# wondras/ld-decode

Hardware: AMD Instinct MI355X
Metric: RF Msamples/s (40 MSPS NTSC, full RF->.tbc decode) (higher is better)
Workload: dtype f64

## Files before the change

### ld-decode_amd/csrc/abi.inc

```
#include <hip/hip_runtime.h>
#include <algorithm>
#include <chrono>
#include <thread>
#include <cmath>
#include <complex>
#include <cstdio>
#include <cstring>
#include <map>
#include <string>
#include <vector>

namespace {

using namespace ldg;

struct DevBuf {
  void* p = nullptr;
  size_t n = 0;
};

}

static inline comb::CombOpt comb_defaults() {
  comb::CombOpt c;
// ... 801 lines not shown
  return LDG_OK;
}

int ldg_set_capture(ldg_ctx* ctx, const void* data, int64_t nsamples, int fmt, int64_t first_sample,
                    int is_device) {
  if (!ctx || !data || nsamples <= 0 || fmt < 0 || fmt > 3 || first_sample < 0) return LDG_EINVAL;
  if ((fmt == 2 && first_sample % 3) || (fmt == 3 && first_sample % 4)) return LDG_EINVAL;
  LDG_TRY(hipSetDevice(ctx->device));
  if (int rc = ldg_stream_close(ctx)) return rc;
  ctx->cap_ring = 0;
  size_t nbytes;
  switch (fmt) {
    case 0: nbytes = (size_t)nsamples; break;
    case 1: nbytes = (size_t)nsamples * 2; break;
    case 2: nbytes = (size_t)((nsamples + 2) / 3) * 4; break;
    default: nbytes = (size_t)((nsamples + 3) / 4) * 5; break;
  }
  if (is_device) {
    if (ctx->cap_owned) dfree(ctx->cap);
    ctx->cap = (uint8_t*)data;
    ctx->cap_owned = false;
    ctx->cap_alloc = nbytes;
  } else {
    if (!ctx->cap_owned || ctx->cap_alloc < nbytes) {
      if (ctx->cap_owned) dfree(ctx->cap);
      ctx->cap = nullptr;
      int rc = dmalloc(ctx, &ctx->cap, nbytes + 16);
      if (rc) return rc;
      ctx->cap_alloc = nbytes;
      ctx->cap_owned = true;
    }
    LDG_TRY(hipMemcpy(ctx->cap, data, nbytes, hipMemcpyHostToDevice));
  }
  ctx->fmt = fmt;
  ctx->cap_first = first_sample;
  ctx->cap_nsamp = nsamples;
  return LDG_OK;
}

static int stream_prepare(ldg_ctx* ctx, hipStream_t s, int64_t hi);

static int64_t steady_ns() {
  return std::chrono::duration_cast<std::chrono::nanoseconds>(std::chrono::steady_clock::now().time_since_epoch())
      .count();
}
static unsigned long long* span_slot(ldg_ctx* ctx) {
  if (!ctx->prof_on || !ctx->d_span || ctx->span_n >= ldg_ctx::SPAN_MAX) return nullptr;
  ctx->span_issue_ns.push_back(steady_ns());
  return ctx->d_span + 2 * (size_t)ctx->span_n++;
}

static int launch_demod(ldg_ctx* ctx, hipStream_t st, int n, const int32_t* M_) {
  const SysConst C = ctx->C;
  LDG_LAUNCH_ON(st, "demod", ldg_k_demod, n * MAX_BLOCKS_PER_READ, 1024, M_, ctx->d_reads, ctx->cap, ctx->cap_first,
             ctx->cap_nsamp, ctx->cap_ring, ctx->fmt, ctx->tw, ctx->twk, ctx->rf_cur, ctx->fvideo, ctx->f05, ctx->iirtab, ctx->alf, ctx->arf, C, ctx->video, ctx->vread, ctx->vchan,
             ctx->d_status, ctx->d_ospill, ++ctx->park_epoch, ctx->d_stile, ctx->d_aslice,
             ctx->d_sst, ctx->d_sbits, ctx->d_bst, span_slot(ctx));
  return check_launch(ctx, "ldg_k_demod");
}

static int launch_chain(ldg_ctx* ctx, hipStream_t st, int n, const int32_t* M_) {
  const SysConst C = ctx->C;
  if (!(ctx->skip >> 0 & 1)) LDG_LAUNCH_ON(st, "sync_walk", ldg_k_sync_walk, n * SEG_K, 64, M_, ctx->d_reads, ctx->video, ctx->vread, ctx->vchan, C,
             ctx->d_status, ctx->d_npos, ctx->d_npk, ctx->d_nlv, ctx->d_ncnt, ctx->d_stile, ctx->d_sst,
             ctx->d_sbits);
  if (!(ctx->skip >> 1 & 1)) LDG_LAUNCH_ON(st, "sync", ldg_k_sync, n, 64, M_, ctx->d_reads, ctx->video, ctx->vread, ctx->vchan, C, ctx->d_recs,
             ctx->d_peaks, ctx->d_status, ctx->d_npos, ctx->d_npk, ctx->d_nlv, ctx->d_ncnt, ctx->d_stile,
             ctx->d_sst, ctx->d_sbits, (ctx->skip >> 9) & 1);
  if (!(ctx->skip >> 2 & 1)) LDG_LAUNCH_ON(st, "linelocs", ldg_k_linelocs, n, 64, M_, ctx->video, ctx->vread, ctx->vchan, C, ctx->d_recs,
             ctx->d_peaks, ctx->d_lines, ctx->d_bad, ctx->d_sst, ctx->d_sbits);
  const dim3 g_lines((unsigned)(C.frame_lines / 2 + 5), (unsigned)n), g_rows((unsigned)(C.frame_lines / 2 + 1), (unsigned)n);
  if (!(ctx->skip >> 3 & 1)) LDG_LAUNCH_ON(st, "hsync_lines", ldg_k_hsync_lines, g_lines, 64, M_, ctx->video, ctx->vread, ctx->vchan, C,
             ctx->d_recs, ctx->d_lines, ctx->d_bad, ctx->d_reads);
  if (!(ctx->skip >> 4 & 1)) LDG_LAUNCH_ON(st, "hsync_field", ldg_k_hsync_field, n, 256, M_, C, ctx->d_recs, ctx->d_lines, ctx->d_bad);
  if (!(ctx->skip >> 5 & 1)) LDG_LAUNCH_ON(st, "philips", ldg_k_philips, n, 192, M_, ctx->video, ctx->vread, ctx->vchan, C, ctx->d_recs,
             ctx->d_lines, ctx->d_reads);
  if (int rc = check_launch(ctx, "field kernels")) return rc;
  if (ctx->system == 0) {
    for (int pass = 0; pass < 2; pass++) {
      if (!(ctx->skip >> 6 & 1)) LDG_LAUNCH_ON(st, "burst_lines", ldg_k_burst_lines, g_lines, 64, M_, ctx->video, ctx->vread, ctx->vchan, C,
                 ctx->d_recs, ctx->d_lines, ctx->d_blevel, pass, ctx->d_bst, ctx->d_reads);
      if (!(ctx->skip >> 7 & 1)) LDG_LAUNCH_ON(st, "burst_field", ldg_k_burst_field, n, 64, M_, ctx->video, ctx->vread, ctx->vchan,
                 ctx->d_recs, ctx->d_lines, ctx->d_blevel, C, pass, ctx->d_bst, ctx->d_reads);
    }
  } else {
    LDG_LAUNCH_ON(st, "pilot_lines", ldg_k_pilot_lines, g_lines, 64, M_, ctx->video, ctx->vread, ctx->vchan, C,
               ctx->d_recs, ctx->d_lines, ctx->d_scratch, ctx->d_reads);
    LDG_LAUNCH_ON(st, "pilot_field", ldg_k_pilot_field, n, 256, M_, ctx->d_recs, ctx->d_lines, C, ctx->d_scratch,
               ctx->d_reads);
  }
  if (!(ctx->skip >> 8 & 1)) {
    if (C.hz_ire_r != 0.0)
      LDG_LAUNCH_ON(st, "final_lines", ldg_k_final_lines, g_rows, FINAL_NT, M_, ctx->video, ctx->vread, ctx->vchan, C,
                    ctx->d_recs, ctx->d_lines, ctx->d_blevel, ctx->d_pic, ctx->pic_stride, ctx->d_reads);
    else
      LDG_LAUNCH_ON(st, "final_lines", ldg_k_final_lines_div, g_rows, FINAL_NT, M_, ctx->video, ctx->vread, ctx->vchan, C,
                    ctx->d_recs, ctx->d_lines, ctx->d_blevel, ctx->d_pic, ctx->pic_stride, ctx->d_reads);
  }
  if (int rc = check_launch(ctx, "tbc kernels")) return rc;
  return LDG_OK;
}

struct HostProf {
  bool on = getenv("LDG_HOSTPROF") != nullptr;
  std::chrono::steady_clock::time_point t0 = std::chrono::steady_clock::now(), t = t0;
  char buf[512];
  int len = 0;
// ... 144 lines not shown
    ctx->rf_tab[ci] = nullptr;
    ctx->rf_cap[ci] = 0;
    if (int rc = dmalloc(ctx, &ctx->rf_tab[ci], (size_t)want * BLOCKLEN)) return rc;
    ctx->rf_cap[ci] = want;
  }
  ctx->rf_cur = ctx->rf_tab[ci];
  if (ctx->cs && (ctx->stages & 1)) {
    int64_t hi = 0;
    for (int i = 0; i < n; i++) {
      const int64_t w = (full && (full[i] & LDG_READ_PROBE)) ? probe_halfwin(ctx->C) : 0;
      hi = std::max(hi, nr[i].s0 + (int64_t)(nr[i].n_blocks - 1) * BLOCKSTEP + BLOCKLEN + w);
    }
    if (int rc = stream_prepare(ctx, s, hi)) return rc;
  }
  ReadDesc* hpr = (ReadDesc*)(ctx->h_probe + (size_t)ci * R * (sizeof(ReadDesc) + sizeof(int32_t)));
  int32_t* hps = (int32_t*)(hpr + R);
  int np = 0;
  if (full)
    for (int i = 0; i < n; i++) {
      if (!(full[i] & LDG_READ_PROBE)) continue;
      ReadDesc pr = nr[i];
      const int64_t r0 = nr[i].readsample - PROBE_C;
      if (!(ctx->stages & 1) || r0 - BLOCKCUT < ctx->cap_first ||
          r0 - BLOCKCUT + BLOCKLEN > ctx->cap_first + ctx->cap_nsamp) {
        full[i] &= (uint8_t)~LDG_READ_PROBE;
        continue;
      }
      read_geometry(pr, r0);
      pr.end = r0 + BLOCKSTEP + 64;
      pr.n_out = (int32_t)(pr.end - pr.s0 + 1);
      pr.n_blocks = 1;
      pr.n_audio = (int32_t)((pr.end - pr.s0) / AUDIO_DIV1 + 1);
      pr.n_audio2 = pr.n_audio / AUDIO_DIV2;
      pr.vcut = 0;
      pr.acut1 = pr.acut2 = ACUT_NONE;
      hpr[np] = pr;
      hps[np++] = smap[i];
    }
  int32_t* dps = ctx->d_psm + (size_t)ci * R;
  hipStream_t sp = ctx->sprep;
  if (call.demod_recorded) LDG_TRY(hipStreamWaitEvent(sp, call.ev_demod, 0));
  LDG_LAUNCH_ON(sp, "new_reads", ldg_k_new_reads, (n + 255) / 256, 256, hnr, hsm, n, dsm, ctx->d_reads, ctx->d_status);
  if (np) LDG_LAUNCH_ON(sp, "new_reads", ldg_k_new_reads, (np + 255) / 256, 256, hpr, hps, np, dps, ctx->d_preads,
                        ctx->d_status);
    LDG_LAUNCH_ON(sp, "rf_table", ldg_k_rf_table, dim3(BLOCKLEN / 256, (unsigned)tm.size()), 256, ctx->rfvideo, ctx->mtf,
                  ctx->mtf_logabs, ctx->mtf_arg, htm, ctx->rf_cur);
  if (int rc = check_launch(ctx, "ldg_k_rf_table")) return rc;
  LDG_TRY(hipEventRecord(call.ev_prep, sp));
  LDG_TRY(hipStreamWaitEvent(s, call.ev_prep, 0));
  if (ctx->frames_recorded && ctx->frames_demod) LDG_TRY(hipStreamWaitEvent(s, ctx->ev_frames, 0));
  hp_.mark("prep");
  if (np && (ctx->stages & 1)) {
    const SysConst C = ctx->C;
    LDG_LAUNCH_ON(s, "demod_probe", ldg_k_demod_probe, np, 1024, dps, ctx->d_preads, ctx->cap, ctx->cap_first,
                  ctx->cap_nsamp, ctx->cap_ring, ctx->fmt, ctx->tw, ctx->twk, ctx->rf_cur, ctx->fvideo, ctx->f05, ctx->iirtab,
                  ctx->alf, ctx->arf, C, ctx->video, ctx->vread, ctx->vchan,
                  ctx->d_status, ctx->d_ospill, ++ctx->park_epoch, ctx->d_stile, ctx->d_aslice, ctx->d_sst,
                  ctx->d_sbits, ctx->d_bst, nullptr);
    LDG_LAUNCH_ON(s, "probe_pick", ldg_k_probe_pick, np, 64, dps, ctx->d_preads, ctx->d_reads, ctx->d_status,
                  ctx->d_sst, ctx->d_sbits, C, probe_halfwin(C));
    if (int rc = check_launch(ctx, "ldg_k_probe_pick")) return rc;
    ctx->probes += np;
  }
  const int ng = (ctx->stages & 4) ? std::max(1, std::min(ctx->nsub, n / 4)) : 0;
  auto group = [&](int g, int& i0, int& m) {
    i0 = (int)((int64_t)n * g / ng);
    m = (int)((int64_t)n * (g + 1) / ng) - i0;
  };
  if (ctx->stages & 1)
    if (int rc = launch_demod(ctx, s, n, dsm)) return rc;
  hp_.mark("demod");
  LDG_TRY(hipEventRecord(call.ev_demod, s));
  call.demod_recorded = true;
  LDG_TRY(hipStreamWaitEvent(ctx->sa, call.ev_demod, 0));
  if (ctx->audio_recorded) LDG_TRY(hipStreamWaitEvent(ctx->sa, ctx->ev_audio, 0));
  if (ctx->stages & 2) LDG_LAUNCH_ON(ctx->sa, "audio1", ldg_k_audio1, n * MAX_BLOCKS_PER_READ, A1_T, dsm, ctx->d_reads,
                                     ctx->tw, ctx->C, ctx->d_aslice, ctx->audio1, ctx->a1read, ctx->a1chan, ctx->d_status);
  if (ctx->stages & 2) LDG_LAUNCH_ON(ctx->sa, "audio2", ldg_k_audio2, n * AUDIO2_WG, 1024, dsm, ctx->d_reads, ctx->tw, ctx->lpf2, ctx->audio1,
                ctx->a1read, ctx->a1chan, ctx->audio2, ctx->a2read, ctx->a2chan, ctx->d_status);
  if (int rc = check_launch(ctx, "ldg_k_audio2")) return rc;
  LDG_TRY(hipEventRecord(call.ev_done[0], ctx->sa));
  hp_.mark("audio");
  int nd = 1;
  for (int g = 0; g < ng; g++) {
    int i0, m;
    group(g, i0, m);
    if (m <= 0) continue;
    hipStream_t st = ctx->sub[g];
    LDG_TRY(hipStreamWaitEvent(st, call.ev_demod, 0));
    if (ctx->frames_recorded) LDG_TRY(hipStreamWaitEvent(st, ctx->ev_frames, 0));
    if (ctx->audio_recorded) LDG_TRY(hipStreamWaitEvent(st, ctx->ev_audio, 0));
    if (int rc = launch_chain(ctx, st, m, dsm + i0)) return rc;
    LDG_TRY(hipEventRecord(call.ev_done[nd++], st));
  hp_.mark("chain");
  }
  call.ndone = nd;
  for (int k = 0; k < nd; k++) LDG_TRY(hipStreamWaitEvent(ctx->srec, call.ev_done[k], 0));
  call.seq = ++ctx->seq;
  LDG_LAUNCH_ON(ctx->srec, "recs_out", ldg_k_recs_out, 1, 256, ctx->d_recs, dsm, n, ctx->d_reads,
                ctx->h_recs_pin + (size_t)ci * R,
                ctx->h_done + ci, call.seq);
  LDG_TRY(hipEventRecord(call.ev_copied, ctx->srec));
  hp_.mark("rec");
  call.n = n;
  call.smap = smap;
  for (int i = 0; i < n; i++) {
    ctx->h_reads[smap[i]] = nr[i];
// ... 831 lines not shown
  if (ctx->pal_state) {
    const double init2[2] = {-1.0, -1.0};
    LDG_TRY(hipMemcpy(ctx->pal_state, init2, sizeof(init2), hipMemcpyHostToDevice));
    ctx->pal_scur = 0;
  }
  return LDG_OK;
}

int ldg_comb_set_state(ldg_ctx* ctx, double aburstlev) {
  if (!ctx) return LDG_EINVAL;
  LDG_TRY(hipSetDevice(ctx->device));
  if (int rc = comb_quiesce(ctx)) return rc;
  if (int rc = comb_alloc(ctx)) return rc;
  LDG_TRY(hipMemcpy(ctx->comb_state, &aburstlev, sizeof(double), hipMemcpyHostToDevice));
  return LDG_OK;
}

int ldg_demod_isolated_ex(ldg_ctx* ctx, int n, const int32_t* slots, int iters, int variant, double* ms_per_launch) {
  if (!ctx || !slots || n <= 0 || n > ctx->max_reads || iters <= 0 || !ms_per_launch) return LDG_EINVAL;
  if (variant != 0 && variant != 1) return LDG_EINVAL;
  for (int i = 0; i < n; i++)
    if (slots[i] < 0 || slots[i] >= ctx->max_reads || !ctx->live[slots[i]]) return LDG_EINVAL;
  LDG_TRY(hipSetDevice(ctx->device));
  LDG_TRY(hipDeviceSynchronize());
  if (!ctx->d_isomap) {
    if (int rc = dmalloc(ctx, &ctx->d_isomap, (size_t)ctx->max_reads)) return rc;
  }
  LDG_TRY(hipMemcpy(ctx->d_isomap, slots, (size_t)n * sizeof(int32_t), hipMemcpyHostToDevice));
  std::vector<int32_t> st_h((size_t)ctx->max_reads);
  LDG_TRY(hipMemcpy(st_h.data(), ctx->d_status, st_h.size() * sizeof(int32_t), hipMemcpyDeviceToHost));
  for (int i = 0; i < n; i++)
    if (st_h[slots[i]] == FS_EOF) { ctx->err = "demod_isolated: a read lies outside the resident capture"; return LDG_ESTATE; }
  if (!ctx->rf_cur) { ctx->err = "demod_isolated: no decode yet"; return LDG_ESTATE; }
  int nt = 1;
  for (int i = 0; i < n; i++) nt = std::max(nt, ctx->h_reads[slots[i]].filt_slot + 1);
  if (ctx->rf_iso_cap < nt) {
    dfree(ctx->rf_iso);
    ctx->rf_iso = nullptr;
    ctx->rf_iso_cap = 0;
    if (int rc = dmalloc(ctx, &ctx->rf_iso, (size_t)nt * BLOCKLEN)) return rc;
    ctx->rf_iso_cap = nt;
  }
  for (int t = 0; t < nt; t++)
    LDG_TRY(hipMemcpy(ctx->rf_iso + (size_t)t * BLOCKLEN, ctx->rf_cur, BLOCKLEN * sizeof(double2),
                      hipMemcpyDeviceToDevice));
  const SysConst C = ctx->C;
  hipStream_t st = ctx->stream;
  std::vector<hipEvent_t> ev(2 * (size_t)iters, nullptr);
  int rc = LDG_OK;
  auto step = [&](hipError_t e) { if (!rc && e != hipSuccess) { ctx->err = hipGetErrorString(e); rc = LDG_EDEVICE; } };
  for (auto& e : ev) step(hipEventCreate(&e));
  for (int k = 0; k < iters && !rc; k++) {
    step(hipEventRecord(ev[2 * k], st));
    (variant ? ldg_k_demod_iso_cut : ldg_k_demod_iso)<<<n * MAX_BLOCKS_PER_READ, 1024, 0, st>>>(
          ctx->d_isomap, ctx->d_reads, ctx->cap, ctx->cap_first, ctx->cap_nsamp, ctx->cap_ring, ctx->fmt, ctx->tw, ctx->twk,
          ctx->rf_iso, ctx->fvideo, ctx->f05, ctx->iirtab, ctx->alf, ctx->arf, C,
          ctx->video, ctx->vread, ctx->vchan, ctx->d_status, ctx->d_ospill,
          ++ctx->park_epoch, ctx->d_stile, ctx->d_aslice, ctx->d_sst, ctx->d_sbits, ctx->d_bst, nullptr);
    step(hipEventRecord(ev[2 * k + 1], st));
  }
  if (!rc) rc = check_launch(ctx, variant ? "ldg_k_demod_iso_cut" : "ldg_k_demod_iso");
  if (!rc) step(hipStreamSynchronize(st));
  double tot = 0;
  for (int k = 0; k < iters && !rc; k++) {
    float ms = 0;
    step(hipEventElapsedTime(&ms, ev[2 * k], ev[2 * k + 1]));
    tot += ms;
  }
  if (!rc) {
    *ms_per_launch = tot / iters;
    step(hipMemcpy(st_h.data(), ctx->d_status, st_h.size() * sizeof(int32_t), hipMemcpyDeviceToHost));
    for (int i = 0; i < n && !rc; i++)
      if (st_h[slots[i]] == FS_EOF) { ctx->err = "demod_isolated: a read returned FS_EOF"; rc = LDG_ESTATE; }
  }
  for (auto& e : ev)
    if (e) (void)hipEventDestroy(e);
  return rc;
}

int ldg_demod_isolated(ldg_ctx* ctx, int n, const int32_t* slots, int iters, double* ms_per_launch) {
  return ldg_demod_isolated_ex(ctx, n, slots, iters, 0, ms_per_launch);
}

int ldg_sync(ldg_ctx* ctx) {
  if (!ctx) return LDG_EINVAL;
  LDG_TRY(hipSetDevice(ctx->device));
  for (hipStream_t st : {ctx->stream2, ctx->scomb, ctx->stream, ctx->stream_b, ctx->sa, ctx->sout, ctx->srec, ctx->sprep}) LDG_TRY(hipStreamSynchronize(st));
  for (int k = 0; k < ctx->nsub; k++) LDG_TRY(hipStreamSynchronize(ctx->sub[k]));
  ctx->comb_pending = false;
  ctx->out_head = ctx->out_n = 0;
  prof_collect(ctx);
  return LDG_OK;
}

int ldg_comb_async(ldg_ctx* ctx, int n) {
  if (!ctx || n < 0 || n > ctx->max_frames) return LDG_EINVAL;
  if (!ctx->have_filters) { ctx->err = "comb: set the filters (the system) first"; return LDG_ESTATE; }
  if (n == 0) return LDG_OK;
  if (ctx->C.system == 0) return ldg_comb_ntsc_async(ctx, n);
  LDG_TRY(hipSetDevice(ctx->device));
  if (int rc = pal_alloc(ctx)) return rc;
  hipStream_t c = ctx->scomb;
  const int b = ctx->fb;
  LDG_TRY(hipStreamWaitEvent(c, ctx->ev_frames, 0));
  if (int rc = pal_launch(ctx, c, ctx->frame_buf(b), n)) return rc;
  LDG_TRY(hipEventRecord(ctx->ev_fbuf[b], c));
  ctx->fbuf_recorded[b] = true;
// ... 721 lines not shown
```

### ld-decode_amd/csrc/demod.hip

```cpp
#include <hip/hip_runtime.h>
#include <type_traits>
#include "common.hpp"
#include "fft8k.hpp"
#include "iir.hpp"
#include "chan.hpp"
#include "tail.hpp"
#include "sample.hpp"

using namespace ldg;

namespace {

constexpr int T = 1024;
constexpr int M = HALF;

__device__ __forceinline__ double2 rsplit(double2 A, double2 B, double2 w) {
  const double2 e = make_double2(0.5 * (A.x + B.x), 0.5 * (A.y - B.y));
  const double2 d = make_double2(A.x - B.x, A.y + B.y);
  const double2 o = make_double2(0.5 * d.y, -0.5 * d.x);
  return cadd(e, cmul(w, o));
}

__device__ __forceinline__ double2 cmerge(double2 Pk, double2 Pkp, double2 w) {
  const double2 e = make_double2(0.5 * (Pk.x + Pkp.x), 0.5 * (Pk.y - Pkp.y));
// ... 37 lines not shown
  } else if (z < 252) {
    p = 32 + (z - 248);
    pp = 39 - (z - 248);
  } else if (z < 255) {
    p = z - 251;
    pp = 8 - p;
  } else if (z == 255) {
    return {0, 0, M};
  } else {
    return {4, 4, 4};
  }
  return {p, pp, pp};
}

static_assert(sizeof(double2) * HALF > 160 * 1024 / 2, "demod workgroups must not share a CU");
__device__ __forceinline__ int cu_slot() {
  const unsigned hw = __builtin_amdgcn_s_getreg((31 << 11) | 4);
  const unsigned xcc = __builtin_amdgcn_s_getreg((31 << 11) | 20);
  return (int)(((xcc & 7u) << 8) | (((hw >> 13) & 7u) << 5) | (((hw >> 12) & 1u) << 4) | ((hw >> 8) & 15u));
}

__device__ __forceinline__ int fresh(int tid) { asm volatile("" : "+v"(tid)); return tid; }

__device__ __forceinline__ bool pair_live(int tid, int c) { return c < 4 || tid == 0; }

__device__ __forceinline__ double2 tw_mirror(double2 w) { return make_double2(-w.x, w.y); }

#ifdef LDG_PROBE
constexpr int kProbe = LDG_PROBE;
#else
constexpr int kProbe = 0;
#endif
#ifdef LDG_PROBE_NOSTORE
constexpr bool kProbeNoStore = true;
#else
constexpr bool kProbeNoStore = false;
#endif

__device__ __forceinline__ void st_pair(double* a, double2 z) {
  typedef double v2d __attribute__((ext_vector_type(2)));
  const v2d zv = {z.x, z.y};
  __builtin_nontemporal_store(zv, reinterpret_cast<v2d*>(a));
}
__device__ __forceinline__ void st_park(double2* a, double2 z) { *a = z; }
__device__ __forceinline__ unsigned long long* park_owner(double2* ospill) {
  return reinterpret_cast<unsigned long long*>(ospill + (int64_t)PARK_TOTAL * M);
}
__device__ __forceinline__ int uni(int v) { return __builtin_amdgcn_readfirstlane(v); }
template <class T> __device__ __forceinline__ T* at32(T* base, int i) {
  using B = std::conditional_t<std::is_const<T>::value, const char, char>;
  return reinterpret_cast<T*>(reinterpret_cast<B*>(base) + (uint32_t)i * (uint32_t)sizeof(T));
}

__device__ __forceinline__ void store_wave(char* ob, uint32_t voff, int lo, int l2, double2 z, int copylen) {
  double* const a = reinterpret_cast<double*>(ob + voff);
  if (lo >= BLOCKCUT && lo + 127 < BLOCKCUT + copylen) {
    st_pair(a, z);
  } else if (lo + 127 >= BLOCKCUT && lo < BLOCKCUT + copylen) {
    const int p = lo + l2;
    const bool in0 = p >= BLOCKCUT && p < BLOCKCUT + copylen;
    const bool in1 = p + 1 >= BLOCKCUT && p + 1 < BLOCKCUT + copylen;
    if (in0 && in1) *reinterpret_cast<double2*>(a) = z;
    else if (in0) a[0] = z.x;
    else if (in1) a[1] = z.y;
  }
}

struct LaneStore {
  uint32_t voff;
  int wlo;
  int l2;
};
__device__ __forceinline__ LaneStore lane_store(int t) { return {16u * (uint32_t)t, uni(2 * (t & ~63)), 2 * (t & 63)}; }
__device__ __forceinline__ void store_q(double* o, LaneStore ls, int q, double2 z, int copylen) {
  store_wave(reinterpret_cast<char*>(o) + 16384 * q, ls.voff, ls.wlo + 2048 * q, ls.l2, z, copylen);
}

__device__ __forceinline__ void store_chan(const double2* sx, double* o, int t, int copylen) {
  if (kProbeNoStore) return;
  const LaneStore ls = lane_store(t);
#pragma unroll
  for (int q = 0; q < 8; q++) {
    const int m = t + 1024 * q;
    store_q(o, ls, q, sx[SWC(m)], copylen);
  }
}

__device__ __forceinline__ bool am_beats32(double v, int vi, double b, int bi) {
  const bool vn = v != v, bn = b != b;
  if (vn || bn) return vn && (!bn || vi < bi);
  return v > b || (v == b && vi < bi);
}

__constant__ double c_atan64[65] = {
    0.0, 0.015623728620476831, 0.031239833430268277, 0.046840712915969654,
    0.06241880999595735, 0.0779666338315423, 0.09347678115858947, 0.1089419569898658,
    0.12435499454676144, 0.13970887428916365, 0.15499674192394097, 0.1702119252854744,
    0.18534794999569476, 0.2003985538258785, 0.21535769969773805, 0.23021958727684372,
    0.24497866312686414, 0.2596296294082575, 0.2741674511196588, 0.2885873618940774,
    0.3028848683749714, 0.31705575320914703, 0.3310960767041321, 0.34500217720710513,
    0.35877067027057225, 0.3723984466767542, 0.38588266939807375, 0.39922076957525254,
    0.4124104415973873, 0.42544963737004227, 0.43833655985795783, 0.4510696559885235,
    0.4636476090008061, 0.4760693303227612, 0.48833395105640554, 0.5004408131472942,
    0.5123894603107377, 0.5241796287829132, 0.5358112379604637, 0.5472843809874369,
    0.5585993153435624, 0.5697564534829784, 0.5807563535676704, 0.5915997103351114,
    0.6022873461349642, 0.6128202021652414, 0.6231993299340659, 0.6334258829691446,
// ... 44 lines not shown
}

__device__ __forceinline__ void merge_pairs(const CBuf x, const double2* __restrict__ twk,
                                            const double2* __restrict__ G, int tid, const Pairs& D) {
  tid = fresh(tid);
#pragma unroll
  for (int c = 0; c < 5; c++) {
    if (!pair_live(tid, c)) continue;
    const Slot sl = slot_of(tid, c);
    const double2 wk = *at32(twk, sl.p);
    const double2 Pk = cmul(D.a[c], *at32(G, sl.p));
    const double2 Pkp = cmul(D.b[c], *at32(G, sl.gp));
    x[sl.p] = cmerge(Pk, Pkp, wk);
    if (sl.pp != sl.p) x[sl.pp] = cmerge(Pkp, Pk, tw_mirror(wk));
  }
}

}

#ifdef LDG_STAMPS
constexpr int LDG_STAMP_BLOCKS = 8192;
__device__ unsigned long long g_stamps[LDG_STAMP_BLOCKS][32];
#define STAMP(i)                                                                   \
  do {                                                                             \
    __syncthreads();                                                               \
    if (threadIdx.x == 0 && blockIdx.x < LDG_STAMP_BLOCKS)                         \
      g_stamps[blockIdx.x][i] = __builtin_readcyclecounter();                      \
  } while (0)
#else
#define STAMP(i) \
  do {           \
  } while (0)
#endif

#define LDG_DEMOD_ARG_LIST(P, V, L)                                                                    \
  P(const int32_t, smap) P(const ReadDesc, reads) P(const uint8_t, cap) V(int64_t, cap_first)         \
  V(int64_t, cap_nsamp) V(int64_t, ring) V(int, fmt) P(const double2, tw) P(const double2, twk)       \
  P(const double2, rf_filt) P(const double2, g_video) P(const double2, g_05) P(const double, iir)     \
  P(const double2, a_lfilt) P(const double2, a_rfilt) V(SysConst, C) P(double, video)                 \
  V(int64_t, vread_stride) V(int64_t, vchan_stride) P(int32_t, status) P(double2, ospill)             \
  V(unsigned long long, park_epoch) P(SyncTile, stiles) P(double2, aslice) P(double, sst)             \
  P(uint32_t, sbits) P(double4, bst) L(unsigned long long, span)
#define LDG_DEMOD_PARAMS LDG_KERNEL_PARAMS(LDG_DEMOD_ARG_LIST)
struct DemodKargs {
  LDG_KARG_FIELDS(LDG_DEMOD_ARG_LIST)
};
#define DK(name) LDG_KARG(DemodKargs, name)
#define DKP(name) LDG_KARG_PTR(DemodKargs, name)
static_assert(alignof(SysConst) == 8 && offsetof(DemodKargs, fmt) == 48 && offsetof(DemodKargs, tw) == 56 &&
                  offsetof(DemodKargs, C) == 120 && offsetof(DemodKargs, video) == 120 + sizeof(SysConst) &&
                  offsetof(DemodKargs, span) == 208 + sizeof(SysConst) && sizeof(DemodKargs) == 216 + sizeof(SysConst),
              "DemodKargs is the kernels' argument list");
#define LDG_DEMOD_ARGS LDG_KERNEL_ARGS(LDG_DEMOD_ARG_LIST)
template <bool CUT, bool PROBE = false>
__device__ __forceinline__ void demod_body(LDG_DEMOD_PARAMS) {
  __shared__ double2 s_x[M];
  __shared__ uint16_t s_bits[BLOCKLEN / 16];
  __shared__ double2 s_tw[TW_LDS_N];
  __shared__ IIRAux s_aux;
  __shared__ double s_atan[65];
  const CBuf X_{s_x};
  const int tid = threadIdx.x;
  if (tid < 65) s_atan[tid] = c_atan64[tid];
  s_tw[tw_lds_pos(tid)] = tw[2 * tid];
  const TwLds twl{s_tw};
  const FftLane fl = fft_lane(tid);
  STAMP(0);
  if (unsigned long long* const span = DKP(span); span && tid == 0)
    atomicMax(&span[0], ~(unsigned long long)__builtin_amdgcn_s_memrealtime());
  const int slot = PROBE ? smap[blockIdx.x] : smap[blockIdx.x / MAX_BLOCKS_PER_READ];
  const int b = PROBE ? 0 : blockIdx.x % MAX_BLOCKS_PER_READ;
  const ReadDesc rd = reads[slot];
  if (b >= rd.n_blocks) return;

  const int64_t i0 = rd.s0 + (int64_t)b * BLOCKSTEP;
  const int off = b * BLOCKSTEP;
  const int copylen = (off + (BLOCKLEN - BLOCKCUT) > rd.n_out) ? rd.n_out - off : BLOCKSTEP;
  int64_t rel0 = i0 - cap_first;
  if (rel0 < 0 || rel0 + BLOCKLEN > cap_nsamp) {
    if (tid == 0) DKP(status)[slot] = FS_EOF;
    return;
  }
  if (ring) {
    const int spg = fmt == 2 ? 3 : fmt == 3 ? 4 : 1, bpg = fmt == 1 ? 2 : fmt == 2 ? 4 : fmt == 3 ? 5 : 1;
    const int64_t g = i0 / spg;
    cap += (g * bpg) % ring;
    rel0 = i0 - g * spg;
  }
  auto vout = [&](int ch) {
    return DKP(video) + (int64_t)slot * DK(vread_stride) + off - BLOCKCUT + (int64_t)ch * DK(vchan_stride);
  };
  const double2* F = rf_filt + (int64_t)rd.filt_slot * BLOCKLEN;
  __shared__ int s_park;
  const int my_cu = cu_slot();
  unsigned long long* const owners = park_owner(ospill);
  const unsigned long long my_tag = (park_epoch << 32) | (unsigned long long)blockIdx.x;
  int my_park = -1;
  if (tid == 0) {
    if (atomicCAS(owners + my_cu, 0ull, my_tag) == 0ull) my_park = my_cu;
    for (int e = 0; e < PARK_EXTRA && my_park < 0; e++) {
      const int u = PARK_SLOTS + ((my_cu + e) & (PARK_EXTRA - 1));
      if (atomicCAS(owners + u, 0ull, my_tag) == 0ull) my_park = u;
    }
    s_park = my_park;
  }
  constexpr double TAU = 6.283185307179586;

  if (fmt == 0 || fmt == 1) {
    double x[16];
    if (fmt == 0) {
      uint4 w;
      __builtin_memcpy(&w, at32(cap + rel0, 16 * tid), 16);
      const uint32_t wd[4] = {w.x, w.y, w.z, w.w};
#pragma unroll
      for (int i = 0; i < 16; i++) x[i] = (double)((wd[i >> 2] >> (8 * (i & 3))) & 0xffu);
    } else {
      uint4 w[2];
      __builtin_memcpy(w, at32(reinterpret_cast<const int16_t*>(cap) + rel0, 16 * tid), 32);
      const uint32_t wd[8] = {w[0].x, w[0].y, w[0].z, w[0].w, w[1].x, w[1].y, w[1].z, w[1].w};
#pragma unroll
      for (int i = 0; i < 16; i++) x[i] = (double)(int16_t)(wd[i >> 1] >> (16 * (i & 1)));
    }
#pragma unroll
    for (int r = 0; r < 8; r++) X_[8 * tid + r] = make_double2(x[2 * r], x[2 * r + 1]);
  } else {
#pragma unroll
    for (int q = 0; q < 8; q++) {
      const int m = tid + T * q;
      X_[m] = make_double2(load_sample(cap, fmt, rel0 + 2 * m), load_sample(cap, fmt, rel0 + 2 * m + 1));
    }
  }
  STAMP(1);
  if (!(kProbe & 8)) fft8k_dif<false>(s_x, tw, twl, tid, fl);
  else __syncthreads();
  STAMP(2);
  const int park_id = uni(s_park);
  const bool park_lost = park_id < 0;
  double2* const park = ospill + (int64_t)(park_lost ? PARK_SCRATCH : park_id) * M;
  auto finish = [&] {
    if (tid == 0 && park_lost) DKP(status)[slot] = FS_MIGRATED;
    if (unsigned long long* const span = DKP(span); span && tid == 0)
      atomicMax(&span[1], (unsigned long long)__builtin_amdgcn_s_memrealtime());
  };

  {
    Pairs X;
    if (!(kProbe & 64)) split_pairs(X_, twk, tid, X);
    else for (int c = 0; c < 5; c++) { X.a[c] = X_[tid + 1024 * c]; X.b[c] = X.a[c]; }
    if (!(CUT && a1_block_dead(b, rd.acut1))) {
      const int t = fresh(tid);
      const int a0 = DK(C).audio_lo0;
      const bool mir = t >= 512;
      const int k = mir ? a0 + 1 + (t - 512) : a0 + t;
      const int j = mir ? a0 + 1024 - k : t;
      double2 xk = rsplit(X_[dr_pos(k)], X_[dr_pos(M - k)], *at32(tw, k));
      if (mir) xk = conj2(xk);
      const double2 al = cmul(xk, *at32(DKP(a_lfilt), j)), ar = cmul(xk, *at32(DKP(a_rfilt), j));
      double2* as = DKP(aslice) + ((int64_t)slot * MAX_BLOCKS_PER_READ + b) * 2048;
      *at32(as, j) = al;
      *at32(as + 1024, j) = ar;
    }
    __syncthreads();
    const int t = fresh(tid);
#pragma unroll
    for (int c = 0; c < 5; c++) {
      if (!pair_live(t, c) || (kProbe & 16)) continue;
      const Slot sl = slot_of(t, c);
      auto Fv = [&](int i) { return (kProbe & 128) ? make_double2(1.0 + i * 1e-9, 0.5) : *at32(F, i); };
      const double2 wk = *at32(twk, sl.p);
      const double2 yk = cmul(X.a[c], Fv(sl.p));
      const double2 yk2 = cmul(conj2(X.b[c]), Fv(M + sl.p));
      X_[sl.p] = cadd(yk, yk2);
      if (!(kProbe & 256)) {
        const double2 o = cmulc(csub(yk, yk2), wk);
        st_park(at32(park, SW(sl.p)), o);
      }
      if (sl.pp != sl.p) {
        const double2 ykp = cmul(X.b[c], Fv(sl.pp));
        const double2 ykp2 = cmul(conj2(X.a[c]), Fv(M + sl.pp));
        X_[sl.pp] = cadd(ykp, ykp2);
        if (!(kProbe & 256)) st_park(at32(park, SW(sl.pp)), cmulc(csub(ykp, ykp2), tw_mirror(wk)));
      }
    }
  }

  STAMP(3);
  double the[8], tho[8];
#pragma clang loop unroll(disable)
  for (int h = 0; h < 2; h++) {
    STAMP(4 + 2 * h);
    if (h == 1 && tid == 0 && my_park >= 0)
      __hip_atomic_store(owners + my_park, 0ull, __ATOMIC_RELAXED, __HIP_MEMORY_SCOPE_AGENT);
    double2 zr[8];
    fft8k_dit<true, true>(s_x, tw, twl, tid, zr, fl);
    if (h == 0) {
      asm volatile("s_waitcnt vmcnt(0)" ::: "memory");
      __syncthreads();
      const int t = fresh(tid);
      const int wbase = __builtin_amdgcn_readfirstlane(t & ~63);
#pragma unroll
      for (int i = 0; i < 8; i++)
        __builtin_amdgcn_global_load_lds((const void*)at32(park + T * i, t),
                                         (__attribute__((address_space(3))) void*)(s_x + T * i + wbase), 16, 0, 0);
    }
    STAMP(5 + 2 * h);
#pragma unroll
    for (int q = 0; q < 8; q++) {
      const double2 z = zr[q];
      const double a = (kProbe & 1) ? z.y * 0.5 + z.x : kFastAtan2 ? fast_atan2(z.y, z.x, s_atan) : atan2(z.y, z.x);
      if (h) tho[q] = a;
      else the[q] = a;
    }
    asm volatile("s_waitcnt vmcnt(0)" ::: "memory");
    __syncthreads();

  }
  double* ph = reinterpret_cast<double*>(s_x);
#pragma unroll
  for (int q = 0; q < 8; q++) ph[tid + T * q] = tho[q];
  __syncthreads();

  STAMP(8);
  {
    const double hzk = DK(C).freq_hz / TAU;
    double d0[8], d1[8];
#pragma unroll
    for (int q = 0; q < 8; q++) {
      const int m = tid + T * q;
      const double prev = m ? ph[m - 1] : 0.0;
      d0[q] = m ? fold_tau(the[q] - prev) * hzk : 0.0;
      d1[q] = fold_tau(tho[q] - the[q]) * hzk;
    }
    __syncthreads();
#pragma unroll
    for (int q = 0; q < 8; q++) X_[tid + T * q] = make_double2(d0[q], d1[q]);
  }
  STAMP(9);
  fft8k_dif<false>(s_x, tw, twl, tid, fl);
  STAMP(10);
  Pairs D;
  if (!(kProbe & 64)) split_pairs(X_, twk, tid, D);
  else for (int c = 0; c < 5; c++) { D.a[c] = X_[tid + 1024 * c]; D.b[c] = D.a[c]; }
  __syncthreads();
  STAMP(11);

  const double inv = 1.0 / (double)M;
  double pl1, pt1, p151, p311;
  double2* sx = s_x;
  {
    if (!(kProbe & 32)) merge_pairs(X_, twk, DKP(g_05), tid, D);
    STAMP(12);
    double2 zr[8];
    fft8k_dit<true, true>(s_x, tw, twl, tid, zr, fl);
    STAMP(13);
    const int t = fresh(tid);
    pl1 = *at32(iir + IIR_P1, t & 63);
    pt1 = *at32(iir + IIR_P1, t);
    p151 = *at32(iir + IIR_P1, scan_d15(t & 63));
    p311 = *at32(iir + IIR_P1, scan_d31(t & 63));
    double* o = vout(CH_05) - BLOCKCUT_END;
    const double sync_lo = DK(C).sync_lo, sync_hi = DK(C).sync_hi;
    LaneStore ls = lane_store(t);
    ls.wlo -= BLOCKCUT_END;
    const bool st05 = !kProbeNoStore && !(CUT && (int64_t)off >= rd.vcut);
#pragma unroll
    for (int q = 0; q < 8; q++) {
      const int m = t + T * q;
      const double v0 = zr[q].x * inv, v1 = zr[q].y * inv;
      if (st05) store_q(o, ls, q, make_double2(v0, v1), copylen);
      const uint32_t f0 = (v0 >= sync_lo && v0 <= sync_hi) ? 1u : 0u;
      const uint32_t f1 = (v1 >= sync_lo && v1 <= sync_hi) ? 1u : 0u;
      int xb = (int)((f0 | (f1 << 1)) << (2 * (t & 7)));
      xb |= __builtin_amdgcn_mov_dpp(xb, 0x111, 0xf, 0xf, true);
      xb |= __builtin_amdgcn_mov_dpp(xb, 0x112, 0xf, 0xf, true);
      xb |= __builtin_amdgcn_mov_dpp(xb, 0x114, 0xf, 0xf, true);
      if ((t & 7) == 7) s_bits[m >> 3] = (uint16_t)xb;
    }
  }
  __syncthreads();
  STAMP(14);
  {
    const int t = fresh(tid);
    const uint32_t cur = s_bits[(t + 2) & 1023], prv = (uint32_t)s_bits[(t + 1) & 1023] >> 15;
    double y[IIR_CHUNK];
    double st_in = 0.0;
    if (!(kProbe & 4)) iir1_bits(cur, prv, iir, &s_aux, t, pl1, pt1, p151, p311, y, &st_in);
    else for (int i = 0; i < IIR_CHUNK; i++) y[i] = (double)((cur >> i) & 1) * pl1;
    const int64_t cbase = (int64_t)slot * CHUNKS_PER_SLOT + (off >> 4) - BLOCKCUT / 16;
    if (16 * t >= BLOCKCUT && 16 * t < BLOCKCUT + copylen) {
      *at32(DKP(sst) + cbase, t) = st_in;
      *at32(DKP(sbits) + cbase, t) = cur | (prv << 16);
    }
    {
      const int j = (t >> 1) - 32, hf = t & 1;
      const int ntile = (copylen + 31) / 32;
      double v = -__builtin_inf();
      int vi = 0x7fffffff;
      const int n0 = 32 * j;
      if (j >= 0 && j < ntile) {
#pragma unroll
        for (int i = 0; i < IIR_CHUNK; i++) {
          const int e = 16 * hf + i;
          if (e < copylen - 32 * j && am_beats32(y[i], n0 + e, v, vi)) { v = y[i]; vi = n0 + e; }
        }
      }
      const double ov = __shfl_xor(v, 1);
      const int oi = __shfl_xor(vi, 1);
      if (am_beats32(ov, oi, v, vi)) { v = ov; vi = oi; }
      if (j >= 0 && j < ntile && hf == 0) {
        SyncTile tt;
        tt.v = v;
        tt.idx = vi == 0x7fffffff ? 0x7fffffffffffffffLL : (int64_t)off + vi;
        *at32(DKP(stiles) + ((int64_t)slot * STILE_PER_SLOT + (off >> 5) - 32), t >> 1) = tt;
      }
    }
  }
  STAMP(15);
  if (CUT && (int64_t)off >= rd.vcut) {
    finish();
    return;
  }
  double4 mlb, mtb, m15b, m31b;
  {
    if (!(kProbe & 32)) merge_pairs(X_, twk, DKP(g_video), tid, D);
    STAMP(16);
    double2 zr[8];
    if (!(kProbe & 2)) fft8k_dit<true, true>(s_x, tw, twl, tid, zr, fl);
    else { __syncthreads(); for (int q = 0; q < 8; q++) zr[q] = s_x[tid + 1024 * q]; __syncthreads(); }
    STAMP(17);
    const int t = fresh(tid);
    mlb = iir2_pow(iir + IIR_MB, t & 63);
    mtb = iir2_pow(iir + IIR_MB, t);
    m15b = iir2_pow(iir + IIR_MB, scan_d15(t & 63));
    m31b = iir2_pow(iir + IIR_MB, scan_d31(t & 63));
    double* o = vout(CH_DEMOD);
    const LaneStore ls = lane_store(t);
#pragma unroll
    for (int q = 0; q < 8; q++) {
      const int m = t + T * q;
      const double2 z = make_double2(zr[q].x * inv, zr[q].y * inv);
      sx[SWC(m)] = z;
      if (!kProbeNoStore) store_q(o, ls, q, z, copylen);
    }
  }
  __syncthreads();
  STAMP(18);
  {
    const int t = fresh(tid);
    double x[IIR_CHUNK];
#pragma unroll
    for (int c = 0; c < 8; c++) {
      const double2 z = sx[SWC(8 * t + c)];
      x[2 * c] = z.x;
      x[2 * c + 1] = z.y;
    }
    const double2 h = sx[SWC((8 * t - 1) & (M - 1))];
    double y[IIR_CHUNK];
    double2 s_in = make_double2(0.0, 0.0);
    if (!(kProbe & 4)) iir2(x, h.y, h.x, iir + 3, iir + IIR_MB, &s_aux, t, mlb, mtb, m15b, m31b, y, &s_in);
    if (16 * t >= BLOCKCUT && 16 * t < BLOCKCUT + copylen) {
      const int64_t cbase = (int64_t)slot * CHUNKS_PER_SLOT + (off >> 4) - BLOCKCUT / 16;
      *at32(DKP(bst) + cbase, t) = make_double4(s_in.x, s_in.y, h.y, h.x);
    }
    if (DK(C).n_chan > 4) {
      double2 p_in;
      iir2(x, h.y, h.x, iir + 8, iir + IIR_MP, &s_aux, t, iir2_pow(iir + IIR_MP, t & 63), iir2_pow(iir + IIR_MP, t),
           iir2_pow(iir + IIR_MP, scan_d15(t & 63)), iir2_pow(iir + IIR_MP, scan_d31(t & 63)), y, &p_in);
#pragma unroll
      for (int c = 0; c < 8; c++) sx[SWC(8 * t + c)] = make_double2(y[2 * c], y[2 * c + 1]);
      __syncthreads();
      store_chan(sx, vout(CH_PILOT), t, copylen);
    }
  }
  STAMP(19);
  finish();
}

extern "C" __global__ __launch_bounds__(1024) void ldg_k_demod(LDG_DEMOD_PARAMS) { demod_body<true>(LDG_DEMOD_ARGS); }

extern "C" __global__ __launch_bounds__(1024) void ldg_k_demod_iso(LDG_DEMOD_PARAMS) { demod_body<false>(LDG_DEMOD_ARGS); }
extern "C" __global__ __launch_bounds__(1024) void ldg_k_demod_iso_cut(LDG_DEMOD_PARAMS) { demod_body<true>(LDG_DEMOD_ARGS); }

constexpr int PROBE_C = BLOCKSTEP / 2;

extern "C" __global__ __launch_bounds__(1024) void ldg_k_demod_probe(LDG_DEMOD_PARAMS) {
  demod_body<true, true>(LDG_DEMOD_ARGS);
}

extern "C" __global__ __launch_bounds__(64) void ldg_k_probe_pick(const int32_t* __restrict__ psm,
                                                                 const ReadDesc* __restrict__ preads,
                                                                 ReadDesc* __restrict__ reads,
                                                                 int32_t* __restrict__ status,
                                                                 const double* __restrict__ sst,
                                                                 const uint32_t* __restrict__ sbits, SysConst C,
                                                                 int halfwin) {
  const int slot = psm[blockIdx.x];
  const int lane = threadIdx.x;
  const bool eof = status[slot] == FS_EOF;
  const SyncSrc ds(sst, sbits, slot, C);
  double best = -1.0;
  int bi = 0x7fffffff;
  if (!eof) {
    for (int o = PROBE_C - halfwin + lane; o <= PROBE_C + halfwin; o += 64) {
      const double v = ds[o];
      if (v > best) { best = v; bi = o; }
    }
  }
#pragma unroll
  for (int m = 1; m < 64; m <<= 1) {
    const double ov = __shfl_xor(best, m);
    const int oi = __shfl_xor(bi, m);
    if (ov > best || (ov == best && oi < bi)) { best = ov; bi = oi; }
  }
  if (lane == 0) {
    if (!eof && best > 0.2) {
      ReadDesc r = reads[slot];
      const int64_t start = preads[slot].readsample + bi;
      r.readsample = start;
      r.end = start + READLEN + 1;
      r.s0 = start > BLOCKCUT ? start - BLOCKCUT : 0;
      r.n_out = (int32_t)(r.end - r.s0 + 1);
      r.n_blocks = (int32_t)((r.end - r.s0 + BLOCKSTEP - 1) / BLOCKSTEP);
      r.n_audio = (int32_t)((r.end - r.s0) / AUDIO_DIV1 + 1);
      r.n_audio2 = r.n_audio / AUDIO_DIV2;
      const TailPlan tp = tail_plan(r.n_audio, r.n_audio2, r.vcut);
      r.acut1 = tp.acut1;
      r.acut2 = tp.acut2;
      if (r.n_out <= MAX_NOUT && r.n_blocks <= MAX_BLOCKS_PER_READ) reads[slot] = r;
    }
    status[slot] = 0;
  }
}

constexpr int A1_T = 256;
constexpr int A1_H = A1_T / 2;
constexpr int A1_P = 1024 / A1_H;
extern "C" __global__ __launch_bounds__(A1_T) void ldg_k_audio1(
    const int32_t* __restrict__ smap, const ReadDesc* __restrict__ reads, const double2* __restrict__ tw, SysConst C,
    const double2* __restrict__ aslice, double* __restrict__ audio1, int64_t aread_stride, int64_t achan_stride,
    const int32_t* __restrict__ status) {
// ... 155 lines not shown
```

Baseline: 24970.

## Specialize demod kernel by packed-format and pilot channel template flags

Result: no change. 24950 (-0.1%).

```diff
diff --git a/ld-decode_amd/csrc/abi.inc b/ld-decode_amd/csrc/abi.inc
--- a/ld-decode_amd/csrc/abi.inc
+++ b/ld-decode_amd/csrc/abi.inc
@@ -877,7 +877,7 @@
 
 static int launch_demod(ldg_ctx* ctx, hipStream_t st, int n, const int32_t* M_) {
   const SysConst C = ctx->C;
-  LDG_LAUNCH_ON(st, "demod", ldg_k_demod, n * MAX_BLOCKS_PER_READ, 1024, M_, ctx->d_reads, ctx->cap, ctx->cap_first,
+  LDG_LAUNCH_ON(st, "demod", demod_kernel(DEMOD_PIPE, ctx->fmt, C.n_chan), n * MAX_BLOCKS_PER_READ, 1024, M_, ctx->d_reads, ctx->cap, ctx->cap_first,
              ctx->cap_nsamp, ctx->cap_ring, ctx->fmt, ctx->tw, ctx->twk, ctx->rf_cur, ctx->fvideo, ctx->f05, ctx->iirtab, ctx->alf, ctx->arf, C, ctx->video, ctx->vread, ctx->vchan,
              ctx->d_status, ctx->d_ospill, ++ctx->park_epoch, ctx->d_stile, ctx->d_aslice,
              ctx->d_sst, ctx->d_sbits, ctx->d_bst, span_slot(ctx));
@@ -1128,7 +1128,7 @@
   hp_.mark("prep");
   if (np && (ctx->stages & 1)) {
     const SysConst C = ctx->C;
-    LDG_LAUNCH_ON(s, "demod_probe", ldg_k_demod_probe, np, 1024, dps, ctx->d_preads, ctx->cap, ctx->cap_first,
+    LDG_LAUNCH_ON(s, "demod_probe", demod_kernel(DEMOD_PROBE, ctx->fmt, C.n_chan), np, 1024, dps, ctx->d_preads, ctx->cap, ctx->cap_first,
                   ctx->cap_nsamp, ctx->cap_ring, ctx->fmt, ctx->tw, ctx->twk, ctx->rf_cur, ctx->fvideo, ctx->f05, ctx->iirtab,
                   ctx->alf, ctx->arf, C, ctx->video, ctx->vread, ctx->vchan,
                   ctx->d_status, ctx->d_ospill, ++ctx->park_epoch, ctx->d_stile, ctx->d_aslice, ctx->d_sst,
@@ -2066,7 +2066,7 @@
   for (auto& e : ev) step(hipEventCreate(&e));
   for (int k = 0; k < iters && !rc; k++) {
     step(hipEventRecord(ev[2 * k], st));
-    (variant ? ldg_k_demod_iso_cut : ldg_k_demod_iso)<<<n * MAX_BLOCKS_PER_READ, 1024, 0, st>>>(
+    demod_kernel(variant ? DEMOD_ISO_CUT : DEMOD_ISO, ctx->fmt, C.n_chan)<<<n * MAX_BLOCKS_PER_READ, 1024, 0, st>>>(
           ctx->d_isomap, ctx->d_reads, ctx->cap, ctx->cap_first, ctx->cap_nsamp, ctx->cap_ring, ctx->fmt, ctx->tw, ctx->twk,
           ctx->rf_iso, ctx->fvideo, ctx->f05, ctx->iirtab, ctx->alf, ctx->arf, C,
           ctx->video, ctx->vread, ctx->vchan, ctx->d_status, ctx->d_ospill,
diff --git a/ld-decode_amd/csrc/demod.hip b/ld-decode_amd/csrc/demod.hip
--- a/ld-decode_amd/csrc/demod.hip
+++ b/ld-decode_amd/csrc/demod.hip
@@ -113,6 +113,16 @@
   return reinterpret_cast<T*>(reinterpret_cast<B*>(base) + (uint32_t)i * (uint32_t)sizeof(T));
 }
 
+__device__ __forceinline__ double sample_r30(const uint8_t* gb, uint32_t u) {
+  const uint32_t w = u / 3u;
+  return (double)((*at32(reinterpret_cast<const uint32_t*>(gb), (int)w) >> (10u * (u - 3u * w))) & 0x3ffu);
+}
+__device__ __forceinline__ double sample_lds(const uint8_t* gb, uint32_t u) {
+  const uint32_t k = u & 3u;
+  const uint8_t* const b = at32(gb, (int)(5u * (u >> 2) + k));
+  return (double)(((((uint32_t)b[0] << 8) | b[1]) >> (6u - 2u * k)) & 0x3ffu);
+}
+
 __device__ __forceinline__ void store_wave(char* ob, uint32_t voff, int lo, int l2, double2 z, int copylen) {
   double* const a = reinterpret_cast<double*>(ob + voff);
   if (lo >= BLOCKCUT && lo + 127 < BLOCKCUT + copylen) {
@@ -263,7 +273,7 @@
                   offsetof(DemodKargs, span) == 208 + sizeof(SysConst) && sizeof(DemodKargs) == 216 + sizeof(SysConst),
               "DemodKargs is the kernels' argument list");
 #define LDG_DEMOD_ARGS LDG_KERNEL_ARGS(LDG_DEMOD_ARG_LIST)
-template <bool CUT, bool PROBE = false>
+template <bool CUT, bool PROBE, bool PACKED, bool PILOT>
 __device__ __forceinline__ void demod_body(LDG_DEMOD_PARAMS) {
   __shared__ double2 s_x[M];
   __shared__ uint16_t s_bits[BLOCKLEN / 16];
@@ -293,7 +303,7 @@
     return;
   }
   if (ring) {
-    const int spg = fmt == 2 ? 3 : fmt == 3 ? 4 : 1, bpg = fmt == 1 ? 2 : fmt == 2 ? 4 : fmt == 3 ? 5 : 1;
+    const int spg = !PACKED ? 1 : fmt == 2 ? 3 : 4, bpg = !PACKED ? (fmt == 1 ? 2 : 1) : fmt == 2 ? 4 : 5;
     const int64_t g = i0 / spg;
     cap += (g * bpg) % ring;
     rel0 = i0 - g * spg;
@@ -317,7 +327,7 @@
   }
   constexpr double TAU = 6.283185307179586;
 
-  if (fmt == 0 || fmt == 1) {
+  if constexpr (!PACKED) {
     double x[16];
     if (fmt == 0) {
       uint4 w;
@@ -335,10 +345,16 @@
 #pragma unroll
     for (int r = 0; r < 8; r++) X_[8 * tid + r] = make_double2(x[2 * r], x[2 * r + 1]);
   } else {
-#pragma unroll
-    for (int q = 0; q < 8; q++) {
-      const int m = tid + T * q;
-      X_[m] = make_double2(load_sample(cap, fmt, rel0 + 2 * m), load_sample(cap, fmt, rel0 + 2 * m + 1));
+    const bool r30 = fmt == 2;
+    const int64_t g0 = r30 ? rel0 / 3 : rel0 >> 2;
+    const uint32_t u0 = (uint32_t)(rel0 - g0 * (r30 ? 3 : 4)) + 2u * (uint32_t)tid;
+    const uint8_t* const gb = cap + g0 * (r30 ? 4 : 5);
+    if (r30) {
+#pragma unroll
+      for (int q = 0; q < 8; q++) X_[tid + T * q] = make_double2(sample_r30(gb, u0 + 2u * T * q), sample_r30(gb, u0 + 2u * T * q + 1));
+    } else {
+#pragma unroll
+      for (int q = 0; q < 8; q++) X_[tid + T * q] = make_double2(sample_lds(gb, u0 + 2u * T * q), sample_lds(gb, u0 + 2u * T * q + 1));
     }
   }
   STAMP(1);
@@ -435,9 +451,10 @@
   {
     const double hzk = DK(C).freq_hz / TAU;
     double d0[8], d1[8];
+    const int t = fresh(tid);
 #pragma unroll
     for (int q = 0; q < 8; q++) {
-      const int m = tid + T * q;
+      const int m = t + T * q;
       const double prev = m ? ph[m - 1] : 0.0;
       d0[q] = m ? fold_tau(the[q] - prev) * hzk : 0.0;
       d1[q] = fold_tau(tho[q] - the[q]) * hzk;
@@ -512,7 +529,9 @@
 #pragma unroll
         for (int i = 0; i < IIR_CHUNK; i++) {
           const int e = 16 * hf + i;
-          if (e < copylen - 32 * j && am_beats32(y[i], n0 + e, v, vi)) { v = y[i]; vi = n0 + e; }
+          const bool take = e < copylen - 32 * j && (vi == 0x7fffffff || (v == v && !(y[i] <= v)));
+          v = take ? y[i] : v;
+          vi = take ? n0 + e : vi;
         }
       }
       const double ov = __shfl_xor(v, 1);
@@ -573,7 +592,7 @@
       const int64_t cbase = (int64_t)slot * CHUNKS_PER_SLOT + (off >> 4) - BLOCKCUT / 16;
       *at32(DKP(bst) + cbase, t) = make_double4(s_in.x, s_in.y, h.y, h.x);
     }
-    if (DK(C).n_chan > 4) {
+    if constexpr (PILOT) {
       double2 p_in;
       iir2(x, h.y, h.x, iir + 8, iir + IIR_MP, &s_aux, t, iir2_pow(iir + IIR_MP, t & 63), iir2_pow(iir + IIR_MP, t),
            iir2_pow(iir + IIR_MP, scan_d15(t & 63)), iir2_pow(iir + IIR_MP, scan_d31(t & 63)), y, &p_in);
@@ -587,16 +606,31 @@
   finish();
 }
 
-extern "C" __global__ __launch_bounds__(1024) void ldg_k_demod(LDG_DEMOD_PARAMS) { demod_body<true>(LDG_DEMOD_ARGS); }
-
-extern "C" __global__ __launch_bounds__(1024) void ldg_k_demod_iso(LDG_DEMOD_PARAMS) { demod_body<false>(LDG_DEMOD_ARGS); }
-extern "C" __global__ __launch_bounds__(1024) void ldg_k_demod_iso_cut(LDG_DEMOD_PARAMS) { demod_body<true>(LDG_DEMOD_ARGS); }
+#define LDG_DEMOD_KERNEL(NAME, CUT, PROBE, PACKED, PILOT)                                   \
+  extern "C" __global__ __launch_bounds__(1024) void NAME(LDG_DEMOD_PARAMS) {                \
+    demod_body<CUT, PROBE, PACKED, PILOT>(LDG_DEMOD_ARGS);                                   \
+  }
+#define LDG_DEMOD_KERNELS(SUF, PACKED, PILOT)                                \
+  LDG_DEMOD_KERNEL(ldg_k_demod##SUF, true, false, PACKED, PILOT)             \
+  LDG_DEMOD_KERNEL(ldg_k_demod_iso##SUF, false, false, PACKED, PILOT)        \
+  LDG_DEMOD_KERNEL(ldg_k_demod_iso_cut##SUF, true, false, PACKED, PILOT)     \
+  LDG_DEMOD_KERNEL(ldg_k_demod_probe##SUF, true, true, PACKED, PILOT)
+LDG_DEMOD_KERNELS(, false, false)
+LDG_DEMOD_KERNELS(_packed, true, false)
+LDG_DEMOD_KERNELS(_pal, false, true)
+LDG_DEMOD_KERNELS(_packed_pal, true, true)
+
+using DemodKernel = void (*)(LDG_DEMOD_PARAMS);
+enum DemodKind { DEMOD_PIPE = 0, DEMOD_ISO = 1, DEMOD_ISO_CUT = 2, DEMOD_PROBE = 3 };
+static DemodKernel demod_kernel(DemodKind kind, int fmt, int n_chan) {
+#define LDG_DEMOD_ROW(SUF) {ldg_k_demod##SUF, ldg_k_demod_iso##SUF, ldg_k_demod_iso_cut##SUF, ldg_k_demod_probe##SUF}
+  static const DemodKernel tab[4][4] = {LDG_DEMOD_ROW(), LDG_DEMOD_ROW(_packed), LDG_DEMOD_ROW(_pal),
+                                        LDG_DEMOD_ROW(_packed_pal)};
+#undef LDG_DEMOD_ROW
+  return tab[(fmt >= 2 ? 1 : 0) + (n_chan > 4 ? 2 : 0)][kind];
+}
 
 constexpr int PROBE_C = BLOCKSTEP / 2;
-
-extern "C" __global__ __launch_bounds__(1024) void ldg_k_demod_probe(LDG_DEMOD_PARAMS) {
-  demod_body<true, true>(LDG_DEMOD_ARGS);
-}
 
 extern "C" __global__ __launch_bounds__(64) void ldg_k_probe_pick(const int32_t* __restrict__ psm,
                                                                  const ReadDesc* __restrict__ preads,
```
